# arkworks-rs/groth16

Measured on AMD Instinct MI355X. Metric: R1CS constraints/sec (create_proof, BLS12-381), higher is better.
Workload: dtype u32-limb Montgomery integers (Fr 255-bit, Fq 381-bit); 1 GPU; SYN(k=22) synthetic R1CS, 4194302 constraints, FFT domain 2^22, bls12_381, full create_proof (7 NTTs + 4 G1 MSMs + 1 G2 MSM), valid proving key generated on the GPU from seeded toxic waste; curve=bls12_381, log2_domain=22, constraints=4194302, key=valid, witness=resident in HBM at entry (--full: value_incl_h2d holds the PCIe-inclusive rates), parallelism=single-gpu

## Files before the change

### groth16_amd/csrc/api.hip

```cpp
#include "api_types.hpp"
#include "key_load.hpp"
#include "prover.hpp"
#include "proof_glue.hpp"
#include "unit_api.hpp"
#include "srs_setup.hpp"
#include "ceremony.hpp"

namespace {
template <class C>
struct Impl : KeyLoader<C>, Prover<C>, ProofGlue<C>, UnitApi<C> {
    typedef C Curve;
    typedef typename C::Fr Fr;
    typedef typename C::Fq Fq;
    typedef typename C::Fq2 Fq2;
};
}

#define G16_DISPATCH(curve, EXPR)                                             \
    do {                                                                      \
        try {                                                                 \
            if ((curve) == G16_BLS12_381) { typedef Impl<Bls12_381> I; return EXPR; } \
            if ((curve) == G16_BN254) { typedef Impl<Bn254> I; return EXPR; }  \
            return G16_ERR_BAD_ARG;                                           \
        } catch (const std::bad_alloc&) {                                     \
// ... 345 lines not shown
    }
    G16_HIP_TRY(hipSetDevice(ctx->device));
    G16_DISPATCH(ctx->curve, I::pk_load(ctx, view, out));
}

int g16_pk_load_bytes(g16_ctx* ctx, const uint8_t* bytes, uint64_t len, int compressed, int validate, g16_pk** out, void* info,
                      uint64_t info_size) {
    if (out) *out = nullptr;
    if (!ctx || !out || (!bytes && len) || (compressed != 0 && compressed != 1) || validate < 0 || validate > 2) return G16_ERR_BAD_ARG;
    if (!ctx->subs.empty()) {
        g_last_error = "g16_pk_load_bytes: the bytes of a key are loaded whole, on one GPU (a multi-device context takes g16_pk_load)";
        return G16_ERR_BAD_ARG;
    }
    return g16::pk_load_bytes(ctx, ctx->curve, ctx->device, ctx->stream, bytes, len, compressed, validate, out, info, info_size);
}

int g16_pk_load_bucket_shard(g16_ctx* ctx, const g16_pk_view* view, int rank, int world, g16_pk** out) {
    if (!ctx || !view || !out || world < 1 || world > 64 || rank < 0 || rank >= world) return G16_ERR_BAD_ARG;
    if (!ctx->subs.empty()) return G16_ERR_BAD_ARG;
    if (world == 1) return g16_pk_load(ctx, view, out);
    G16_HIP_TRY(hipSetDevice(ctx->device));
    G16_DISPATCH(ctx->curve, I::pk_load(ctx, view, out, world, rank));
}

int g16_pk_rebind_bucket_shard(g16_pk* pk, int rank, int world) {
    if (!pk || world < 1 || world > 64 || rank < 0 || rank >= world || !pk->subs.empty() || !pk->dp) return G16_ERR_BAD_ARG;
    auto rebind = [&](auto* dp) -> int {
        if (dp->c_z == 0 || dp->a_start || dp->b_g1_start || dp->b_g2_start || dp->h_start || dp->l_start) return G16_ERR_BAD_ARG;
        dp->shard_n = world;
        dp->shard_r = rank;
        return G16_OK;
    };
    if (pk->ctx->finprep.key_id == pk->id) pk->ctx->finprep.drop();
    pk->ctx->drop_prepared_sort(pk->id);
    if (pk->curve == G16_BLS12_381) return rebind(static_cast<DevicePk<Bls12_381>*>(pk->dp));
    return rebind(static_cast<DevicePk<Bn254>*>(pk->dp));
}

int g16_pk_get_info(const g16_pk* pk, g16_pk_info* out) {
    if (!pk || !out) return G16_ERR_BAD_ARG;
    memset(out, 0, sizeof(*out));
    const g16_pk* one = pk->subs.empty() ? pk : pk->subs[0];
    if (!one || !one->dp) return G16_ERR_BAD_ARG;
    auto fill = [&](const auto* dp) {
        out->window_bits_z = dp->c_z;
        out->window_bits_h = dp->c_h;
        out->table_fallback = dp->table_fallback;
        out->bucket_shard_rank = dp->shard_r;
        out->bucket_shard_world = dp->shard_n;
        out->device_bytes = dp->table_bytes;
    };
    if (one->curve == G16_BLS12_381) fill(static_cast<const DevicePk<Bls12_381>*>(one->dp));
    else fill(static_cast<const DevicePk<Bn254>*>(one->dp));
    out->n_devices = pk->subs.empty() ? 1 : (int)pk->subs.size();
    return G16_OK;
}

void g16_pk_free(g16_pk* pk) {
    if (!pk) return;
    if (!pk->ctx->subs.empty()) {
        for (g16_pk* sub : pk->subs) g16_pk_free(sub);
        delete pk;
        return;
    }
    if (pk->ctx->finprep.key_id == pk->id) pk->ctx->finprep.drop();
    (void)hipSetDevice(pk->ctx->device);
    pk->ctx->drop_prepared_sort(pk->id);
    if (pk->curve == G16_BLS12_381) Impl<Bls12_381>::pk_free(static_cast<DevicePk<Bls12_381>*>(pk->dp));
    else Impl<Bn254>::pk_free(static_cast<DevicePk<Bn254>*>(pk->dp));
    delete pk;
}

int g16_circuit_load(g16_ctx* ctx, const g16_csr_view abc[3], uint64_t num_inputs, uint64_t num_constraints, uint64_t num_variables,
                     g16_circuit** out) {
    return g16_circuit_load_qap(ctx, abc, num_inputs, num_constraints, num_variables, G16_QAP_LIBSNARK, out);
}

int g16_circuit_qap(const g16_circuit* c) { return c ? c->qap : -1; }

int g16_circuit_load_qap(g16_ctx* ctx, const g16_csr_view abc[3], uint64_t num_inputs, uint64_t num_constraints, uint64_t num_variables,
                         int qap, g16_circuit** out) {
    if (!ctx || !abc || !out) return G16_ERR_BAD_ARG;
    if (qap != G16_QAP_LIBSNARK && qap != G16_QAP_CIRCOM) return G16_ERR_BAD_ARG;
    if (!ctx->subs.empty()) {
        if (qap != G16_QAP_LIBSNARK) {
            g_last_error = "a Circom circuit cannot be loaded on a multi-device context (use one context per GPU and g16_prove_partial)";
            return G16_ERR_BAD_ARG;
        }
        const int n = (int)ctx->subs.size();
        g16_circuit* h = new (std::nothrow) g16_circuit{ctx->curve, ctx, nullptr, 0};
        if (!h) return G16_ERR_OOM;
        h->subs.assign((size_t)n, nullptr);
        const int rc = for_each_device(n, [&](int i) -> int {
            return g16_circuit_load(ctx->subs[(size_t)i], abc, num_inputs, num_constraints, num_variables, &h->subs[(size_t)i]);
        }, serial_loads(ctx));
        if (rc) { g16_circuit_free(h); return rc; }
        h->domain_size = h->subs[0]->domain_size;
        h->num_variables = num_variables;
// ... 727 lines not shown
```

### groth16_amd/csrc/api_types.hpp

```cpp
#pragma once
#include "internal.hpp"
#include "msm_common.hpp"
#include "fp30.hpp"
#include "fixed_base.hpp"
#include <atomic>
#include <chrono>
#include <condition_variable>
#include <future>
#include <mutex>
#include <thread>
#include <new>
#include <type_traits>
#include <dlfcn.h>

namespace g16 {

static thread_local std::string g_last_error;

void set_last_error(const char* what, hipError_t e, const char* file, int line) {
    char buf[512];
    snprintf(buf, sizeof(buf), "%s:%d: %s -> %s", file, line, what, hipGetErrorString(e));
    g_last_error = buf;
}

// ... 65 lines not shown
    hipEvent_t ev_up[8] = {};
    hipStream_t stream_wm = nullptr;
    hipEvent_t ev_dwm = nullptr;
    hipEvent_t ev_heavy[4] = {};
    hipEvent_t ev_edge[8] = {};
    struct Prepared {
        bool valid = false;
        const g16_pk* pk = nullptr;
        uint64_t key_id = 0;
        uint64_t a_start = 0, a_count = 0;
        int c_z = 0;
        const uint64_t* z = nullptr;
        uint64_t n_assign = 0;
        ScalarSort sort_z;
    } prep;
    void drop_prepared_sort(uint64_t id) {
        if (prep.valid && prep.key_id == id) { (void)hipStreamSynchronize(stream2); prep.valid = false; }
    }
    void reset_arena() {
        if (prep.valid) (void)hipStreamSynchronize(stream2);
        arena.reset();
        prep.valid = false;
    }
    hipStream_t red[5];
    Arena arena;
    g16_timings tm;
    g16_srs_timings srs_tm = {};
    double ceremony_ms[6] = {};
    double phase1_ms[5] = {};
    EventTimer t_wm, t_prep_h, t_prep_z, t_bucket[5], t_ntt[2];
    hipEvent_t ev_z = nullptr, ev_h = nullptr, ev_wm = nullptr, ev_done[5] = {};
    struct FinPrep {
        bool valid = false;
        std::future<void> fut;
        std::shared_ptr<void> data;
        uint64_t key_id = 0;
        uint64_t r[4] = {}, s[4] = {};
        bool matches(uint64_t id, const uint64_t* r_, const uint64_t* s_) const {
            return valid && key_id == id && memcmp(r, r_, 32) == 0 && memcmp(s, s_, 32) == 0;
        }
        void drop() {
            if (fut.valid()) fut.wait();
            valid = false;
            data.reset();
            key_id = 0;
        }
    } finprep;
    void* pinned = nullptr;
    size_t pinned_bytes = 0;
    uint64_t* check_z = nullptr;
    size_t check_z_bytes = 0;
    void* check_rec = nullptr;
    std::vector<g16_ctx*> subs;
    std::vector<char> peer;
};

struct DrainOnError {
    g16_ctx* ctx;
    bool armed = true;
    explicit DrainOnError(g16_ctx* c) : ctx(c) {}
    void dismiss() { armed = false; }
    ~DrainOnError() {
        if (!armed) return;
        (void)hipStreamSynchronize(ctx->stream);
        (void)hipStreamSynchronize(ctx->stream2);
        (void)hipStreamSynchronize(ctx->stream3);
        (void)hipStreamSynchronize(ctx->stream_wm);
        (void)hipStreamSynchronize(ctx->stream_h2d);
        for (int i = 0; i < 5; ++i) (void)hipStreamSynchronize(ctx->red[i]);
    }
};

struct g16_dwm;
struct DwmSlot {
    g16_dwm* dwm = nullptr;
    uint64_t *work[3] = {nullptr, nullptr, nullptr}, *recv[3] = {nullptr, nullptr, nullptr}, *h_local = nullptr;
    mutable uint64_t* h_full = nullptr;
    uint64_t* z_dev = nullptr;
};

// ... 76 lines not shown
```

### groth16_amd/csrc/internal.hpp

```cpp
#pragma once
#include <hip/hip_runtime.h>
#include <atomic>
#include <cstdint>
#include <cstdio>
#include <cstring>
#include <string>
#include <vector>
#include "../../include/g16_mi355x.h"
#include "curve.hpp"

namespace g16 {

void set_last_error(const char* what, hipError_t e, const char* file, int line);

#define G16_HIP_TRY(expr)                                                     \
    do {                                                                      \
        hipError_t e__ = (expr);                                              \
        if (e__ != hipSuccess) {                                              \
            ::g16::set_last_error(#expr, e__, __FILE__, __LINE__);            \
            return e__ == hipErrorOutOfMemory ? G16_ERR_OOM : G16_ERR_HIP;    \
        }                                                                     \
    } while (0)

#define G16_TRY(expr)                  \
// ... 168 lines not shown
    uint32_t max_segments = 0;
    uint64_t max_sorted = 0;
};
template <class C> int sort_scalars(const typename C::Fr* d_scalars, uint64_t n, int merged_c, Arena& arena, hipStream_t st, ScalarSort* out,
                                    int shard_n = 1, int shard_r = 0);
static constexpr int COEFF128_SWORDS = 7;
int coeffs128_plan(uint64_t n, MsmPlan* plan);
int sort_digit_planes(const MsmPlan& plan, const uint16_t* planes, uint64_t n, Arena& arena, hipStream_t st, ScalarSort* out);
int msm_slot_layout(const uint32_t* counts, uint32_t M, int R, uint32_t lseg, uint32_t* offsets, uint32_t* nparts, uint32_t* task_off,
                    uint32_t* heavy, uint32_t* block_sums, hipStream_t st);

template <class F>
struct MsmBuffers {
    void* partials = nullptr;
    void* chunk_out = nullptr;
    XYZZ<F>* window_sums = nullptr;
};
template <class F> int msm_bucket_pass(const Affine<F>* d_bases, int64_t shift, uint64_t base_count, const ScalarSort& ss, Arena& arena,
                                       hipStream_t st, MsmBuffers<F>* out, EventTimer* bucket_timer);
template <class F>
struct PassJob {
    const Affine<F>* bases;
    int64_t shift;
    uint64_t base_count;
    const ScalarSort* ss;
    MsmBuffers<F>* out;
};
template <class F> int msm_bucket_pass_batch(const PassJob<F>* jobs, int n, Arena& arena, hipStream_t st, EventTimer* bucket_timer);
template <class F> int msm_reduce(const MsmBuffers<F>& buf, const ScalarSort& ss, hipStream_t st);
template <class F> int msm_reduce_batch(const MsmBuffers<F>* const* bufs, const ScalarSort* const* sorts, int n, hipStream_t st, bool heavy_done);
template <class F> int msm_heavy_reduce(const MsmBuffers<F>& buf, const ScalarSort& ss, hipStream_t st);
template <class F> int msm_heavy_reduce_batch(const MsmBuffers<F>* const* bufs, const ScalarSort* const* sorts, int n, hipStream_t st);
template <class F> int convert_bases(Affine<F>* d_bases, uint64_t n, hipStream_t st);
template <class F> XYZZ<F> fold_windows(const XYZZ<F>* window_sums, const MsmPlan& plan);
template <class F> int build_window_tables(const Affine<F>* d_src, uint64_t n, int c, int W, Affine<F>* d_table, hipStream_t st, void* park = nullptr);
template <class F> size_t window_table_park_bytes(uint64_t n, int W);

template <class C>
int generate_parameters_device(hipStream_t st, Arena& arena, const g16_csr_view abc[3], uint64_t ni, uint64_t nc, uint64_t nv, int qap,
                               const g16_toxic_waste* tw, const uint64_t* g1_gen, const uint64_t* g2_gen, const g16_params_view* out);
template <class C>
int h_query_scalars_host(int qap, uint64_t domain_size, const uint64_t* t, const uint64_t* delta_inverse, uint64_t* out);
template <class C>
int qap_evaluations_host(const g16_csr_view abc[3], uint64_t ni, uint64_t nc, uint64_t nv, const uint64_t* t, uint64_t* a_out, uint64_t* b_out,
                         uint64_t* c_out, uint64_t* zt_out);

int serialize_points(int curve, int g2, int compressed, const uint64_t* points, uint64_t n, uint8_t* out);
int deserialize_points(int curve, int g2, int compressed, const uint8_t* in, uint64_t n, int validate, uint64_t* points_out);
uint64_t serialized_point_size(int curve, int g2, int compressed);

int pk_load_bytes(g16_ctx* ctx, int curve, int device, hipStream_t s, const uint8_t* bytes, uint64_t len, int compressed, int validate,
                  g16_pk** out, void* info_out, uint64_t info_size);

int mad_rate_device(hipStream_t st, double* mad_per_s);
template <class C> int synth_bases_device(int g2, uint64_t seed, uint64_t first, uint64_t n, void* out_dev, hipStream_t st);

}
```

### groth16_amd/csrc/msm.hip

```cpp
#include "internal.hpp"
#include "msm_common.hpp"
#include "fp30.hpp"
#include "acc_store.hpp"
#include "batch_affine.hpp"
#include "window_tables.hpp"
#include <algorithm>
#include <cstdlib>

namespace g16 {

static constexpr int SORT_THREADS = 1024;
static constexpr int RED_THREADS = 64;
static constexpr int WIN_THREADS = 256;
#ifndef G16_REDUCE_G
#define G16_REDUCE_G 8
#endif
static constexpr uint32_t REDUCE_G = G16_REDUCE_G;

struct PlanDev {
    int c, W;
    uint32_t B;
    uint32_t K[10];
    uint32_t shard_n, shard_r, shard_magic;
};

__device__ __forceinline__ bool shard_local_key(const PlanDev& plan, uint32_t* key) {
    if (plan.shard_n <= 1) return true;
    const uint32_t q = __umulhi(*key, plan.shard_magic);
    if (*key - q * plan.shard_n != plan.shard_r) return false;
    *key = q;
    return true;
}

template <class Fr>
__global__ __launch_bounds__(256) void digits_kernel(const Fr* __restrict__ scalars, uint64_t n, PlanDev plan,
                                                     uint16_t* __restrict__ planes) {
    __shared__ uint32_t sw[MSM_SWORDS][256];
    const uint64_t i = (uint64_t)blockIdx.x * 256 + threadIdx.x;
    if (i >= n) return;
    uint32_t s[Fr::N];
// ... 1251 lines not shown
    const MsmPlan& plan = sorts[0]->plan;
    for (int i = 1; i < n; ++i)
        if (sorts[i]->plan.B != plan.B || sorts[i]->plan.groups != plan.groups) return G16_ERR_INTERNAL;
    const uint32_t G = plan.chunk_buckets();
    const uint32_t cpw = plan.B / G;
    size_t lds_heavy, lds_win;
    G16_TRY(reduce_setup<F>(&lds_heavy, &lds_win));
    const auto batch = make_reduce_batch<F>(bufs, sorts, n);
    if (!heavy_done) G16_TRY((msm_heavy_reduce_batch<F>(bufs, sorts, n, st)));
    hipLaunchKernelGGL((bucket_reduce_kernel<F30>), dim3((cpw * plan.groups * F30::LANES_PER_TASK + RED_THREADS - 1) / RED_THREADS, n), dim3(RED_THREADS), 0,
                       st, batch, plan.B, plan.groups, G);
    G16_LAUNCH_CHECK();
    hipLaunchKernelGGL((window_reduce_kernel<F30>), dim3(plan.groups, plan.planes(), n), dim3(WIN_THREADS), lds_win, st, batch, cpw);
    G16_LAUNCH_CHECK();
    return G16_OK;
}

template <class F>
int msm_reduce(const MsmBuffers<F>& buf, const ScalarSort& ss, hipStream_t st) {
    const MsmBuffers<F>* b = &buf;
    const ScalarSort* s = &ss;
    return msm_reduce_batch<F>(&b, &s, 1, st, false);
}

template <class F>
int convert_bases(Affine<F>* d_bases, uint64_t n, hipStream_t st) {
    if (n == 0) return G16_OK;
    hipLaunchKernelGGL((convert_bases30_kernel<F>), dim3((unsigned)((n + 255) / 256)), dim3(256), 0, st, d_bases, n);
    G16_LAUNCH_CHECK();
    return G16_OK;
}

template <class F>
XYZZ<F> fold_windows(const XYZZ<F>* ws, const MsmPlan& plan) {
    const int NP = plan.planes(), bits = plan.chunk_bits();
    auto group_T = [&](int g) -> XYZZ<F> {
        const XYZZ<F>* P = ws + (size_t)g * NP;
        XYZZ<F> hi = XYZZ<F>::identity();
        for (int k = bits - 1; k >= 0; --k) { hi = hi.dbl(); hi.add(P[2 + k]); }
        for (uint32_t b = plan.chunk_buckets(); b > 1; b >>= 1) hi = hi.dbl();
        hi.add(P[0]);
        return hi;
    };
    XYZZ<F> total = XYZZ<F>::identity();
    if (plan.merged) {
        const int Q = plan.groups;
        if (Q > 1) {
            XYZZ<F> run = XYZZ<F>::identity();
            for (int q = Q - 1; q >= 1; --q) { run.add(ws[(size_t)q * NP + 1]); total.add(run); }
            for (uint32_t b = plan.B; b > 1; b >>= 1) total = total.dbl();
        }
        for (int q = 0; q < Q; ++q) total.add(group_T(q));
        if (plan.shard_n > 1) {
            XYZZ<F> plain = XYZZ<F>::identity();
            for (int q = 0; q < Q; ++q) plain.add(ws[(size_t)q * NP + 1]);
            const uint32_t kn = (uint32_t)plan.shard_n, km = (uint32_t)(plan.shard_n - 1 - plan.shard_r);
            total = total.mul_bits(&kn, 7);
            if (km) total.add(plain.mul_bits(&km, 7).neg());
        }
        return total;
    }
    for (int w = plan.W - 1; w >= 0; --w) {
        for (int k = 0; k < plan.c; ++k) total = total.dbl();
        total.add(group_T(w));
    }
    return total;
}

static constexpr int TABLE_MAX_W = 32;
static constexpr int TABLE_THREADS = 128;
static constexpr uint64_t TABLE_CHUNK = (uint64_t)1 << 18;
template <class F30>
__global__ __launch_bounds__(TABLE_THREADS, 2) void build_window_tables_kernel(const Affine<typename F30::Std>* __restrict__ src, uint64_t first,
                                                                              uint64_t count, uint64_t n, int c, int W,
                                                                              Affine<typename F30::Std>* __restrict__ table, uint32_t* __restrict__ park) {
    typedef TableDeviceIO<F30> IO;
    typedef typename IO::W32 W32;
    const uint64_t lane = (uint64_t)blockIdx.x * TABLE_THREADS + threadIdx.x;
    const uint64_t t = lane / F30::LANES_PER_TASK;
    if (t >= count) return;
    const uint64_t i = first + t;
    IO io{reinterpret_cast<const W32*>(src + i), reinterpret_cast<W32*>(table + i), n * 2 * IO::TL::PARTS, park + lane, count * F30::LANES_PER_TASK};
    window_table_task<F30>(io, c, W);
}

// ... 17 lines not shown
    for (uint64_t first = 0; first < n && rc == G16_OK; first += chunk) {
        const uint64_t count = std::min(chunk, n - first);
        const uint64_t lanes = count * F30::LANES_PER_TASK;
        hipLaunchKernelGGL((build_window_tables_kernel<F30>), dim3((unsigned)((lanes + TABLE_THREADS - 1) / TABLE_THREADS)), dim3(TABLE_THREADS), 0, st,
                           d_src, first, count, n, c, W, d_table, park);
        if (hipGetLastError() != hipSuccess) rc = G16_ERR_HIP;
    }
    if (!park_buf) {
        if (hipStreamSynchronize(st) != hipSuccess && rc == G16_OK) rc = G16_ERR_HIP;
        (void)hipFree(park);
    }
    return rc;
}

#define G16_INSTANTIATE_MSM(C)                                                                                               \
    template int convert_bases<typename C::Fq>(Affine<typename C::Fq>*, uint64_t, hipStream_t);                             \
    template int convert_bases<typename C::Fq2>(Affine<typename C::Fq2>*, uint64_t, hipStream_t);                           \
    template int sort_scalars<C>(const typename C::Fr*, uint64_t, int, Arena&, hipStream_t, ScalarSort*, int, int);                   \
    template int build_window_tables<typename C::Fq>(const Affine<typename C::Fq>*, uint64_t, int, int, Affine<typename C::Fq>*, hipStream_t, void*);    \
    template int build_window_tables<typename C::Fq2>(const Affine<typename C::Fq2>*, uint64_t, int, int, Affine<typename C::Fq2>*, hipStream_t, void*); \
    template size_t window_table_park_bytes<typename C::Fq>(uint64_t, int);                                                 \
    template size_t window_table_park_bytes<typename C::Fq2>(uint64_t, int);                                                \
    template int msm_bucket_pass<typename C::Fq>(const Affine<typename C::Fq>*, int64_t, uint64_t, const ScalarSort&, Arena&, \
                                                 hipStream_t, MsmBuffers<typename C::Fq>*, EventTimer*);                      \
    template int msm_bucket_pass<typename C::Fq2>(const Affine<typename C::Fq2>*, int64_t, uint64_t, const ScalarSort&,     \
                                                  Arena&, hipStream_t, MsmBuffers<typename C::Fq2>*, EventTimer*);            \
    template int msm_bucket_pass_batch<typename C::Fq>(const PassJob<typename C::Fq>*, int, Arena&, hipStream_t, EventTimer*);   \
    template int msm_bucket_pass_batch<typename C::Fq2>(const PassJob<typename C::Fq2>*, int, Arena&, hipStream_t, EventTimer*); \
    template int msm_reduce<typename C::Fq>(const MsmBuffers<typename C::Fq>&, const ScalarSort&, hipStream_t);             \
    template int msm_reduce_batch<typename C::Fq>(const MsmBuffers<typename C::Fq>* const*, const ScalarSort* const*, int, hipStream_t, bool); \
    template int msm_heavy_reduce<typename C::Fq>(const MsmBuffers<typename C::Fq>&, const ScalarSort&, hipStream_t);     \
    template int msm_heavy_reduce_batch<typename C::Fq>(const MsmBuffers<typename C::Fq>* const*, const ScalarSort* const*, int, hipStream_t); \
    template int msm_reduce<typename C::Fq2>(const MsmBuffers<typename C::Fq2>&, const ScalarSort&, hipStream_t);           \
    template XYZZ<typename C::Fq> fold_windows<typename C::Fq>(const XYZZ<typename C::Fq>*, const MsmPlan&);               \
    template XYZZ<typename C::Fq2> fold_windows<typename C::Fq2>(const XYZZ<typename C::Fq2>*, const MsmPlan&);

#if G16_MSM_PART == 0
G16_INSTANTIATE_MSM(Bls12_381)
#else
G16_INSTANTIATE_MSM(Bn254)
#endif

}
```

### groth16_amd/csrc/proof_glue.hpp

```cpp
#pragma once
#include "api_types.hpp"

namespace {

template <class C>
struct ProofGlue {
    typedef typename C::Fr Fr;
    typedef typename C::Fq Fq;
    typedef typename C::Fq2 Fq2;
    typedef typename C::G1A G1A;
    typedef typename C::G2A G2A;
    typedef typename C::G1X G1X;
    typedef typename C::G2X G2X;
    static constexpr int L = Fq::N / 2;
    struct FixedPoints {
        G1A alpha_g1, beta_g1, delta_g1, a_query0, b_g1_query0;
        G2A beta_g2, delta_g2, b_g2_query0;
    };
    struct FinalizePrep {
        G1X A0;
        G2X B2;
        G1X C0;
        uint32_t rk[Fr::N], sk[Fr::N];
        bool r_zero;
// ... 41 lines not shown
        G1X h_acc = G1X::identity(), l_acc = G1X::identity(), a_msm = G1X::identity(), b1_msm = G1X::identity();
        G2X b2_msm = G2X::identity();
        for (int i = 0; i < n_parts; ++i) {
            h_acc.add(load_xyzz<G1X>(parts[i].h));
            l_acc.add(load_xyzz<G1X>(parts[i].l));
            a_msm.add(load_xyzz<G1X>(parts[i].a));
            b1_msm.add(load_xyzz<G1X>(parts[i].b_g1));
            b2_msm.add(load_xyzz<G2X>(parts[i].b_g2));
        }
        auto fut_b2 = std::async(std::launch::async, [&]() {
            G2X g2_b = fp.B2;
            g2_b.add(b2_msm);
            return g2_b.to_affine();
        });
        const bool need_rb1 = !fp.r_zero && !b1_msm.is_identity();
        std::future<G1X> fut_rb1;
        if (need_rb1) fut_rb1 = std::async(std::launch::async, [&]() { return mul_window4(b1_msm, fp.rk); });
        G1X g_a = fp.A0;
        g_a.add(a_msm);
        G1X g_c = fp.C0;
        g_c.add(mul_window4(a_msm, fp.sk));
        g_c.add(l_acc);
        g_c.add(h_acc);
        if (need_rb1) g_c.add(fut_rb1.get());
        G1A pa, pc;
        two_to_affine(g_a, g_c, &pa, &pc);
        const G2A pb = fut_b2.get();
        memset(out, 0, sizeof(*out));
        memcpy(out->a, &pa, sizeof(pa));
        memcpy(out->b, &pb, sizeof(pb));
        memcpy(out->c, &pc, sizeof(pc));
        return G16_OK;
    }
    static int finalize_core(const FixedPoints& pk, const g16_partial* parts, int n_parts, const uint64_t* r_, const uint64_t* s_,
                             g16_proof* out, const FixedBaseTable<G1X>* d1 = nullptr, const FixedBaseTable<G2X>* d2 = nullptr) {
        if (n_parts < 1) return G16_ERR_BAD_ARG;
        return finalize_finish(finalize_prepare_core(pk, r_, s_, d1, d2), parts, n_parts, out);
    }
    static FixedPoints fixed_points(const KeyGlue<C>* pk) {
        return {pk->alpha_g1, pk->beta_g1, pk->delta_g1, pk->a_query0, pk->b_g1_query0, pk->beta_g2, pk->delta_g2, pk->b_g2_query0};
    }
    static void ensure_delta_tables(KeyGlue<C>* pk) {
        std::lock_guard<std::mutex> lk(pk->tab_mu);
        if (!pk->tabs_ready.load(std::memory_order_relaxed) && ++pk->finalize_calls >= 2) {
            auto f1 = std::async(std::launch::async, [&]() { pk->delta1_tab.build(G1X::from_affine(pk->delta_g1)); });
            pk->delta2_tab.build(G2X::from_affine(pk->delta_g2));
            f1.get();
            pk->tabs_ready.store(true, std::memory_order_release);
        }
    }
    static const FixedBaseTable<G1X>* table1(const KeyGlue<C>* pk) { return pk->tabs_ready.load(std::memory_order_acquire) ? &pk->delta1_tab : nullptr; }
    static const FixedBaseTable<G2X>* table2(const KeyGlue<C>* pk) { return pk->tabs_ready.load(std::memory_order_acquire) ? &pk->delta2_tab : nullptr; }
    static int prove_finalize_prepare(g16_ctx* ctx, const g16_pk* pkh, const uint64_t* r_, const uint64_t* s_) {
        const std::shared_ptr<KeyGlue<C>> glue = static_cast<const DevicePk<C>*>(pkh->dp)->glue;
        ctx->finprep.drop();
        auto data = std::make_shared<FinalizePrep>();
        ctx->finprep.data = data;
        ctx->finprep.key_id = pkh->id;
        memcpy(ctx->finprep.r, r_, 32);
        memcpy(ctx->finprep.s, s_, 32);
        struct RS { uint64_t r[4], s[4]; } rs;
        memcpy(rs.r, r_, 32);
        memcpy(rs.s, s_, 32);
        ctx->finprep.fut = std::async(std::launch::async, [glue, data, rs]() {
            ensure_delta_tables(glue.get());
            *data = finalize_prepare_core(fixed_points(glue.get()), rs.r, rs.s, table1(glue.get()), table2(glue.get()));
        });
        ctx->finprep.valid = true;
        return G16_OK;
    }
    static int prove_finalize(g16_ctx* ctx, const g16_pk* pkh, const g16_partial* parts, int n_parts, const uint64_t* r_, const uint64_t* s_,
                              g16_proof* out) {
        KeyGlue<C>* pk = static_cast<const DevicePk<C>*>(pkh->dp)->glue.get();
        const double t0 = now_ms();
        if (n_parts < 1) return G16_ERR_BAD_ARG;
        if (ctx->finprep.matches(pkh->id, r_, s_)) {
            ctx->finprep.fut.get();
            const std::shared_ptr<void> keep = ctx->finprep.data;
            ctx->finprep.valid = false;
            G16_TRY(finalize_finish(*static_cast<const FinalizePrep*>(keep.get()), parts, n_parts, out));
        } else {
            ensure_delta_tables(pk);
            G16_TRY(finalize_core(fixed_points(pk), parts, n_parts, r_, s_, out, table1(pk), table2(pk)));
        }
        const double dt = now_ms() - t0;
        ctx->tm.finish_ms += dt;
        ctx->tm.total_ms += dt;
        return G16_OK;
    }
    static int finalize_host(const g16_pk_view* v, const g16_partial* parts, int n_parts, const uint64_t* r_, const uint64_t* s_,
                             g16_proof* out) {
        if (!v->alpha_g1 || !v->beta_g1 || !v->delta_g1 || !v->beta_g2 || !v->delta_g2 || !v->a_query0 || !v->b_g1_query0 ||
            !v->b_g2_query0)
            return G16_ERR_BAD_ARG;
        const FixedPoints fp = {load_pod<G1A>(v->alpha_g1), load_pod<G1A>(v->beta_g1), load_pod<G1A>(v->delta_g1), load_pod<G1A>(v->a_query0),
                                load_pod<G1A>(v->b_g1_query0), load_pod<G2A>(v->beta_g2), load_pod<G2A>(v->delta_g2),
                                load_pod<G2A>(v->b_g2_query0)};
        return finalize_core(fp, parts, n_parts, r_, s_, out);
    }

};

}
```

### groth16_amd/csrc/prover.hpp

```cpp
#pragma once
#include "api_types.hpp"

namespace {

template <class C>
struct Prover {
    typedef typename C::Fr Fr;
    typedef typename C::Fq Fq;
    typedef typename C::Fq2 Fq2;
    typedef typename C::G1A G1A;
    typedef typename C::G2A G2A;
    typedef typename C::G1X G1X;
    typedef typename C::G2X G2X;
    static constexpr int L = Fq::N / 2;
    static int stage_assignment(g16_ctx* ctx, const uint64_t* z, uint64_t n_assign, int on_device, const Fr** d_z) {
        if (on_device) { *d_z = reinterpret_cast<const Fr*>(z); return G16_OK; }
        Fr* buf = nullptr;
        G16_TRY(ctx->arena.alloc_n(n_assign, &buf));
        G16_HIP_TRY(hipMemcpyAsync(buf, z, n_assign * sizeof(Fr), hipMemcpyHostToDevice, ctx->stream));
        *d_z = buf;
        return G16_OK;
    }


    static int prove_partial_prepare(g16_ctx* ctx, const g16_pk* pkh, const g16_circuit* ckh, const uint64_t* z_dev, uint64_t n_assign) {
        const DevicePk<C>* pk = static_cast<const DevicePk<C>*>(pkh->dp);
        const DeviceCircuit<C>* ck = static_cast<const DeviceCircuit<C>*>(ckh->dc);
        if (n_assign != ck->num_variables) return G16_ERR_BAD_LENGTH;
        if (pk->a_start + pk->a_count > n_assign - 1) return G16_ERR_BAD_LENGTH;
        DrainOnError drain(ctx);
        ctx->reset_arena();
        const Fr* d_z = reinterpret_cast<const Fr*>(z_dev);
        ScalarSort ss;
        G16_TRY((sort_scalars<C>(d_z + 1 + pk->a_start, pk->a_count, pk->c_z, ctx->arena, ctx->stream2, &ss, pk->shard_n, pk->shard_r)));
        G16_HIP_TRY(hipEventRecord(ctx->ev_z, ctx->stream2));
        ctx->prep.valid = true;
        ctx->prep.pk = pkh;
        ctx->prep.key_id = pkh->id;
        ctx->prep.a_start = pk->a_start;
        ctx->prep.a_count = pk->a_count;
        ctx->prep.c_z = pk->c_z;
        ctx->prep.z = z_dev;
        ctx->prep.n_assign = n_assign;
        ctx->prep.sort_z = ss;
        drain.dismiss();
        return G16_OK;
    }

    static int prove_partial(g16_ctx* ctx, const g16_pk* pkh, const g16_circuit* ckh, const uint64_t* z, uint64_t n_assign, int on_device,
                             int skip_b_g1, g16_partial* out, const Fr* h_ext = nullptr, uint64_t h_ext_len = 0) {
        const DevicePk<C>* pk = static_cast<const DevicePk<C>*>(pkh->dp);
        const DeviceCircuit<C>* ck = static_cast<const DeviceCircuit<C>*>(ckh->dc);
        hipStream_t s1 = ctx->stream, s2 = ctx->stream2, s3 = ctx->stream3;
        if (n_assign != ck->num_variables) return G16_ERR_BAD_LENGTH;
        const uint64_t n = ck->dom->n, nin = ck->num_inputs;
        const uint64_t m = n_assign - 1, w = n_assign - nin;
        if (pk->a_start + pk->a_count > m || pk->l_start + pk->l_count > w || pk->h_start + pk->h_count > (h_ext ? h_ext_len : n))
            return G16_ERR_BAD_LENGTH;
        if (pk->b_g1_start != pk->a_start || pk->b_g1_count != pk->a_count || pk->b_g2_start != pk->a_start ||
            pk->b_g2_count != pk->a_count)
            return G16_ERR_BAD_ARG;
        memset(out, 0, sizeof(*out));
        const double t_begin = now_ms();
        DrainOnError drain(ctx);
        const bool prepared = ctx->prep.valid && on_device && ctx->prep.pk == pkh && ctx->prep.key_id == pkh->id && ctx->prep.z == z &&
                              ctx->prep.n_assign == n_assign && ctx->prep.a_start == pk->a_start && ctx->prep.a_count == pk->a_count &&
                              ctx->prep.c_z == pk->c_z && ctx->prep.sort_z.plan.shard_n == pk->shard_n &&
                              ctx->prep.sort_z.plan.shard_r == pk->shard_r;
        const ScalarSort prepared_sort = ctx->prep.sort_z;
        if (prepared) ctx->prep.valid = false;
        else ctx->reset_arena();
        const Fr* d_z = nullptr;
        ZUpload up;
        const bool chunked = !on_device && !h_ext && !prepared && !(getenv("G16_UPLOAD_CHUNKED") && atoi(getenv("G16_UPLOAD_CHUNKED")) == 0);
        if (chunked) {
            Fr* buf = nullptr;
            G16_TRY(ctx->arena.alloc_n(n_assign, &buf));
            d_z = buf;
            up.host = z;
            up.copy_stream = ctx->stream_h2d;
            for (int i = 0; i < 8; ++i) up.landed[i] = ctx->ev_up[i];
        } else {
            G16_TRY(stage_assignment(ctx, z, n_assign, on_device, &d_z));
            if (!prepared) G16_HIP_TRY(hipEventRecord(ctx->ev_z, s1));
        }

        const bool overlap_map = !h_ext && getenv("G16_MAP_UNDER_PASSES") != nullptr && atoi(getenv("G16_MAP_UNDER_PASSES")) != 0;
        hipStream_t sm = overlap_map ? ctx->stream_wm : s1;
        Fr* d_h = nullptr;
        ScalarSort sort_h, sort_z, sort_l;
        if (overlap_map && !chunked) G16_HIP_TRY(hipStreamWaitEvent(sm, ctx->ev_z, 0));
        G16_TRY(ctx->t_wm.start(sm));
        if (h_ext) {
            d_h = const_cast<Fr*>(h_ext);
            ctx->t_ntt[0].used = ctx->t_ntt[1].used = false;
// ... 62 lines not shown
        };

        const bool l_covered = pk->l_count == 0 || (pk->l_start + nin - 1 >= pk->a_start &&
                                                    pk->l_start + pk->l_count + nin - 1 <= pk->a_start + pk->a_count);
        {
            hipStream_t sr = short_passes ? ctx->red[4] : s2;
            RoctxRange rr("Compute B in G2");
            if (concurrent) {
                G16_HIP_TRY(hipStreamWaitEvent(sr, ctx->ev_z, 0));
                G16_HIP_TRY(hipStreamWaitEvent(sr, ctx->ev_wm, 0));
                G16_TRY(run_pass(4, pk->b_g2, 0, pk->b_g2_count, sort_z, &buf_b2, sr));
            } else {
                G16_TRY(run_pass(4, pk->b_g2, 0, pk->b_g2_count, sort_z, &buf_b2));
                G16_HIP_TRY(hipStreamWaitEvent(sr, pass_end[4], 0));
            }
            G16_TRY((msm_reduce(buf_b2, sort_z, sr)));
            G16_TRY(copy_out(4, buf_b2, sort_z, sr));
        }
        struct G1Job { int k; MsmBuffers<Fq>* buf; const ScalarSort* ss; };
        G1Job jobs[4];
        int njobs = 0;
        PassJob<Fq> pj[4];
        int pk_of[4], npj = 0;
        double weight[5] = {0, 0, 0, 0, 0};
        auto plans_match = [](const MsmPlan& x, const MsmPlan& y) {
            return x.B == y.B && x.groups == y.groups && x.Lmax == y.Lmax && x.merged == y.merged && x.affine_levels == 0 && y.affine_levels == 0;
        };
        const bool batch_ok = sort_z.plan.affine_levels == 0 || sort_z.max_sorted == 0;
        bool h_in_batch = h_ext != nullptr && batch_ok && plans_match(sort_z.plan, sort_h.plan) && !getenv("G16_PASS_NO_BATCH");
        if (const char* e = getenv("G16_PASS_H_IN_BATCH")) h_in_batch = h_in_batch && atoi(e) != 0;
        int g1_launches = 0;
        bool last_batch = false, early[4] = {false, false, false, false};
        int early_ev[4] = {0, 1, 2, 3};
        auto run_batch = [&]() -> int {
            if (!npj) return G16_OK;
            hipEvent_t b0, b1;
            if (last_end) b0 = last_end;
            else G16_TRY(mark(&b0));
            if (batch_ok && !getenv("G16_PASS_NO_BATCH")) {
                G16_TRY((msm_bucket_pass_batch<Fq>(pj, npj, ctx->arena, s1, nullptr)));
                ++g1_launches;
            } else {
                for (int i = 0; i < npj; ++i) {
                    G16_TRY((msm_bucket_pass<Fq>(pj[i].bases, pj[i].shift, pj[i].base_count, *pj[i].ss, ctx->arena, s1, pj[i].out, nullptr)));
                    ++g1_launches;
                }
            }
            G16_TRY(mark(&b1));
            last_end = b1;
            for (int i = 0; i < npj; ++i) { pass_begin[pk_of[i]] = b0; pass_end[pk_of[i]] = b1; }
            if (!last_batch) {
                const MsmBuffers<Fq>* eb[4];
                const ScalarSort* es[4];
                for (int i = 0; i < npj; ++i) { eb[i] = pj[i].out; es[i] = pj[i].ss; }
                const int k0 = pk_of[0];
                G16_HIP_TRY(hipStreamWaitEvent(ctx->red[k0], b1, 0));
                if (batch_ok) {
                    G16_TRY((msm_heavy_reduce_batch<Fq>(eb, es, npj, ctx->red[k0])));
                } else {
                    for (int i = 0; i < npj; ++i) G16_TRY((msm_heavy_reduce<Fq>(*eb[i], *es[i], ctx->red[k0])));
                }
                G16_HIP_TRY(hipEventRecord(ctx->ev_heavy[k0], ctx->red[k0]));
                for (int i = 0; i < npj; ++i) { early[pk_of[i]] = true; early_ev[pk_of[i]] = k0; }
            }
            npj = 0;
            return G16_OK;
        };
        auto queue_pass = [&](int k, const G1A* bases, int64_t shift, uint64_t count, const ScalarSort& ss, MsmBuffers<Fq>* buf) {
            pj[npj] = PassJob<Fq>{bases, shift, count, &ss, buf};
            pk_of[npj++] = k;
            weight[k] = (double)count;
            jobs[njobs++] = {k, buf, &ss};
        };
        if (l_covered) {
            const int64_t shift = (int64_t)pk->a_start - (int64_t)(nin - 1) - (int64_t)pk->l_start;
            queue_pass(1, pk->l, shift, pk->l_count, sort_z, &buf_l);
        } else {
            G16_TRY((sort_scalars<C>(d_z + nin + pk->l_start, pk->l_count, pk->c_z, ctx->arena, s1, &sort_l, pk->shard_n, pk->shard_r)));
            last_end = nullptr;
            queue_pass(1, pk->l, 0, pk->l_count, sort_l, &buf_l);
            G16_TRY(run_batch());
        }
        { RoctxRange rr("Compute A");
        queue_pass(2, pk->a, 0, pk->a_count, sort_z, &buf_a); }
        if (!skip_b_g1) {
            RoctxRange rr("Compute B in G1");
            queue_pass(3, pk->b_g1, 0, pk->b_g1_count, sort_z, &buf_b1);
        }
        if (!h_in_batch) G16_TRY(run_batch());
        G16_HIP_TRY(hipStreamWaitEvent(s1, ctx->ev_h, 0));
        if (!h_in_batch) last_end = nullptr;
        { RoctxRange rr("Compute C");
        queue_pass(0, pk->h, 0, pk->h_count, sort_h, &buf_h);
        last_batch = true;
        G16_TRY(run_batch()); }
        bool done[4] = {false, false, false, false};
        for (int i = 0; i < njobs; ++i) {
            if (done[i]) continue;
            const MsmBuffers<Fq>* bb[4];
            const ScalarSort* sp[4];
            int idx[4], nb = 0;
            for (int q = i; q < njobs; ++q)
                if (!done[q] && jobs[q].ss->plan.B == jobs[i].ss->plan.B && jobs[q].ss->plan.groups == jobs[i].ss->plan.groups) {
                    bb[nb] = jobs[q].buf; sp[nb] = jobs[q].ss; idx[nb] = q; ++nb;
                    done[q] = true;
                }
            bool any_early = false;
            for (int q = 0; q < nb; ++q) any_early = any_early || early[jobs[idx[q]].k];
            for (int q = 0; q < nb; ++q) {
                if (early[jobs[idx[q]].k]) G16_HIP_TRY(hipStreamWaitEvent(s1, ctx->ev_heavy[early_ev[jobs[idx[q]].k]], 0));
                else if (any_early) G16_TRY((msm_heavy_reduce<Fq>(*bb[q], *sp[q], s1)));
            }
            G16_TRY((msm_reduce_batch<Fq>(bb, sp, nb, s1, any_early)));
            for (int q = 0; q < nb; ++q) G16_TRY(copy_out(jobs[idx[q]].k, *jobs[idx[q]].buf, *jobs[idx[q]].ss, s1));
        }

        double fold_ms = 0.0;
        {
            G16_HIP_TRY(hipEventSynchronize(ctx->ev_done[4]));
            const double t0 = now_ms();
            store_xyzz(out->b_g2, fold_windows<Fq2>(reinterpret_cast<const G2X*>(pin + 4 * SLOT), sort_z.plan));
            fold_ms += now_ms() - t0;
        }
        if (skip_b_g1) store_xyzz(out->b_g1, G1X::identity());
        {
            for (int q = 0; q < njobs; ++q) G16_HIP_TRY(hipEventSynchronize(ctx->ev_done[jobs[q].k]));
            const double t0 = now_ms();
            struct FoldJob { int k; const MsmPlan* plan; uint64_t* dst; };
            const FoldJob fj[4] = {{1, l_covered ? &sort_z.plan : &sort_l.plan, out->l}, {2, &sort_z.plan, out->a}, {3, &sort_z.plan, out->b_g1},
                                   {0, &sort_h.plan, out->h}};
            auto fold_one = [&](const FoldJob& f) { store_xyzz(f.dst, fold_windows<Fq>(reinterpret_cast<const G1X*>(pin + f.k * SLOT), *f.plan)); };
            std::future<void> fut[3];
            int nf = 0;
            for (int q = 0; q < 3; ++q) {
                if (fj[q].k == 3 && skip_b_g1) continue;
                const FoldJob f = fj[q];
                fut[nf++] = std::async(std::launch::async, [&fold_one, f]() { fold_one(f); });
            }
            fold_one(fj[3]);
            for (int q = 0; q < nf; ++q) fut[q].get();
            fold_ms += now_ms() - t0;
        }
        G16_HIP_TRY(hipStreamSynchronize(s1));
        G16_HIP_TRY(hipStreamSynchronize(s2));
        G16_HIP_TRY(hipStreamSynchronize(s3));
        if (overlap_map) G16_HIP_TRY(hipStreamSynchronize(ctx->stream_wm));
        for (int k = 0; k < 5; ++k) G16_HIP_TRY(hipStreamSynchronize(ctx->red[k]));
        drain.dismiss();
        const double t_end = now_ms();

        g16_timings& tm = ctx->tm;
        memset(&tm, 0, sizeof(tm));
        auto span = [&](int k) -> double {
            float t = 0.f;
            return (pass_begin[k] && hipEventElapsedTime(&t, pass_begin[k], ctx->ev_done[k]) == hipSuccess) ? (double)t : 0.0;
        };
        tm.witness_map_ms = ctx->t_wm.ms();
        tm.ntt_ms = ctx->t_ntt[0].ms() + ctx->t_ntt[1].ms();
        tm.scalar_prep_ms = ctx->t_prep_h.ms() + ctx->t_prep_z.ms();
        tm.msm_h_ms = span(0);
        tm.msm_l_ms = span(1);
        tm.msm_a_ms = span(2);
        tm.msm_b_g1_ms = skip_b_g1 ? 0.0 : span(3);
        tm.msm_b_g2_ms = span(4);
        for (int i = 0; i < 5; ++i) {
            float t = 0.f;
            tm.bucket_ms[i] = (pass_begin[i] && pass_end[i] && hipEventElapsedTime(&t, pass_begin[i], pass_end[i]) == hipSuccess) ? (double)t : 0.0;
            double wsum = 0.0;
            for (int q = 0; q < 4; ++q) if (pass_begin[q] == pass_begin[i] && pass_end[q] == pass_end[i]) wsum += weight[q];
            if (i < 4 && wsum > 0.0) tm.bucket_ms[i] *= weight[i] / wsum;
            tm.bucket_pass_ms += tm.bucket_ms[i];
        }
        tm.g1_pass_launches = (double)g1_launches;
        tm.finish_ms = fold_ms;
        tm.total_ms = t_end - t_begin;
        tm.window_bits = sort_z.plan.c;
        tm.windows = sort_z.plan.W;
        return G16_OK;
    }

};
// ... 3 lines not shown
```

Baseline: 66.69 million constraints/s.

## Overlap host window folds and proof glue with remaining GPU MSM work

When the whole key is on one device, the light G1 MSM reductions are now finished and copied out early on the reduce streams. Two worker threads fold the G2 and G1 window sums, with multithreaded fold_windows, and compute the A, B and partial C glue while the H MSM is still running on the GPU. The glue result is cached in a FinCache keyed by key id, r, s and the partial sums, so finalize only adds H and converts C to affine. This adds host threads, more synchronisation complexity and cache-invalidation paths.

```diff
diff --git a/groth16_amd/csrc/api.hip b/groth16_amd/csrc/api.hip
--- a/groth16_amd/csrc/api.hip
+++ b/groth16_amd/csrc/api.hip
@@ -401,6 +401,7 @@
         return G16_OK;
     };
     if (pk->ctx->finprep.key_id == pk->id) pk->ctx->finprep.drop();
+    if (pk->ctx->fincache.key_id == pk->id) pk->ctx->fincache.drop();
     pk->ctx->drop_prepared_sort(pk->id);
     if (pk->curve == G16_BLS12_381) return rebind(static_cast<DevicePk<Bls12_381>*>(pk->dp));
     return rebind(static_cast<DevicePk<Bn254>*>(pk->dp));
@@ -433,6 +434,7 @@
         return;
     }
     if (pk->ctx->finprep.key_id == pk->id) pk->ctx->finprep.drop();
+    if (pk->ctx->fincache.key_id == pk->id) pk->ctx->fincache.drop();
     (void)hipSetDevice(pk->ctx->device);
     pk->ctx->drop_prepared_sort(pk->id);
     if (pk->curve == G16_BLS12_381) Impl<Bls12_381>::pk_free(static_cast<DevicePk<Bls12_381>*>(pk->dp));
diff --git a/groth16_amd/csrc/api_types.hpp b/groth16_amd/csrc/api_types.hpp
--- a/groth16_amd/csrc/api_types.hpp
+++ b/groth16_amd/csrc/api_types.hpp
@@ -121,7 +121,7 @@
     hipEvent_t ev_z = nullptr, ev_h = nullptr, ev_wm = nullptr, ev_done[5] = {};
     struct FinPrep {
         bool valid = false;
-        std::future<void> fut;
+        std::shared_future<void> fut;
         std::shared_ptr<void> data;
         uint64_t key_id = 0;
         uint64_t r[4] = {}, s[4] = {};
@@ -135,6 +135,19 @@
             key_id = 0;
         }
     } finprep;
+    struct FinCache {
+        std::atomic<bool> ready{false};
+        uint64_t key_id = 0;
+        uint64_t r[4] = {}, s[4] = {};
+        g16_partial part = {};
+        uint64_t a[12] = {}, b[24] = {};
+        uint64_t c_part[24] = {};
+        void drop() { ready.store(false, std::memory_order_release); key_id = 0; }
+        bool matches(uint64_t id, const uint64_t* r_, const uint64_t* s_, const g16_partial* p, int n_parts) const {
+            return n_parts == 1 && ready.load(std::memory_order_acquire) && key_id == id && memcmp(r, r_, 32) == 0 && memcmp(s, s_, 32) == 0 &&
+                   memcmp(&part, p, sizeof(g16_partial)) == 0;
+        }
+    } fincache;
     void* pinned = nullptr;
     size_t pinned_bytes = 0;
     uint64_t* check_z = nullptr;
diff --git a/groth16_amd/csrc/internal.hpp b/groth16_amd/csrc/internal.hpp
--- a/groth16_amd/csrc/internal.hpp
+++ b/groth16_amd/csrc/internal.hpp
@@ -224,7 +224,7 @@
 template <class F> int msm_heavy_reduce(const MsmBuffers<F>& buf, const ScalarSort& ss, hipStream_t st);
 template <class F> int msm_heavy_reduce_batch(const MsmBuffers<F>* const* bufs, const ScalarSort* const* sorts, int n, hipStream_t st);
 template <class F> int convert_bases(Affine<F>* d_bases, uint64_t n, hipStream_t st);
-template <class F> XYZZ<F> fold_windows(const XYZZ<F>* window_sums, const MsmPlan& plan);
+template <class F> XYZZ<F> fold_windows(const XYZZ<F>* window_sums, const MsmPlan& plan, int threads = 1);
 template <class F> int build_window_tables(const Affine<F>* d_src, uint64_t n, int c, int W, Affine<F>* d_table, hipStream_t st, void* park = nullptr);
 template <class F> size_t window_table_park_bytes(uint64_t n, int W);
 
diff --git a/groth16_amd/csrc/msm.hip b/groth16_amd/csrc/msm.hip
--- a/groth16_amd/csrc/msm.hip
+++ b/groth16_amd/csrc/msm.hip
@@ -6,6 +6,7 @@
 #include "window_tables.hpp"
 #include <algorithm>
 #include <cstdlib>
+#include <future>
 
 namespace g16 {
 
@@ -1323,7 +1324,7 @@
 }
 
 template <class F>
-XYZZ<F> fold_windows(const XYZZ<F>* ws, const MsmPlan& plan) {
+XYZZ<F> fold_windows(const XYZZ<F>* ws, const MsmPlan& plan, int threads) {
     const int NP = plan.planes(), bits = plan.chunk_bits();
     auto group_T = [&](int g) -> XYZZ<F> {
         const XYZZ<F>* P = ws + (size_t)g * NP;
@@ -1341,7 +1342,20 @@
             for (int q = Q - 1; q >= 1; --q) { run.add(ws[(size_t)q * NP + 1]); total.add(run); }
             for (uint32_t b = plan.B; b > 1; b >>= 1) total = total.dbl();
         }
-        for (int q = 0; q < Q; ++q) total.add(group_T(q));
+        const int nt = threads < 1 ? 1 : (threads > Q ? Q : threads);
+        if (nt > 1) {
+            auto range_T = [&](int t) {
+                XYZZ<F> acc = XYZZ<F>::identity();
+                for (int q = (int)((int64_t)Q * t / nt); q < (int)((int64_t)Q * (t + 1) / nt); ++q) acc.add(group_T(q));
+                return acc;
+            };
+            std::vector<std::future<XYZZ<F>>> fut;
+            for (int t = 1; t < nt; ++t) fut.push_back(std::async(std::launch::async, range_T, t));
+            total.add(range_T(0));
+            for (auto& f : fut) total.add(f.get());
+        } else {
+            for (int q = 0; q < Q; ++q) total.add(group_T(q));
+        }
         if (plan.shard_n > 1) {
             XYZZ<F> plain = XYZZ<F>::identity();
             for (int q = 0; q < Q; ++q) plain.add(ws[(size_t)q * NP + 1]);
@@ -1425,8 +1439,8 @@
     template int msm_heavy_reduce<typename C::Fq>(const MsmBuffers<typename C::Fq>&, const ScalarSort&, hipStream_t);     \
     template int msm_heavy_reduce_batch<typename C::Fq>(const MsmBuffers<typename C::Fq>* const*, const ScalarSort* const*, int, hipStream_t); \
     template int msm_reduce<typename C::Fq2>(const MsmBuffers<typename C::Fq2>&, const ScalarSort&, hipStream_t);           \
-    template XYZZ<typename C::Fq> fold_windows<typename C::Fq>(const XYZZ<typename C::Fq>*, const MsmPlan&);               \
-    template XYZZ<typename C::Fq2> fold_windows<typename C::Fq2>(const XYZZ<typename C::Fq2>*, const MsmPlan&);
+    template XYZZ<typename C::Fq> fold_windows<typename C::Fq>(const XYZZ<typename C::Fq>*, const MsmPlan&, int);              \
+    template XYZZ<typename C::Fq2> fold_windows<typename C::Fq2>(const XYZZ<typename C::Fq2>*, const MsmPlan&, int);
 
 #if G16_MSM_PART == 0
 G16_INSTANTIATE_MSM(Bls12_381)
diff --git a/groth16_amd/csrc/proof_glue.hpp b/groth16_amd/csrc/proof_glue.hpp
--- a/groth16_amd/csrc/proof_glue.hpp
+++ b/groth16_amd/csrc/proof_glue.hpp
@@ -97,6 +97,44 @@
         memcpy(out->c, &pc, sizeof(pc));
         return G16_OK;
     }
+    struct EarlyGlue {
+        G1A a;
+        G2A b;
+        G1X c_part;
+    };
+    static G2A early_b(const FinalizePrep& fp, const G2X& b2_msm) {
+        G2X g2_b = fp.B2;
+        g2_b.add(b2_msm);
+        return g2_b.to_affine();
+    }
+    static void early_ac(const FinalizePrep& fp, const G1X& l_acc, const G1X& a_msm, const G1X& b1_msm, G1A* pa, G1X* c_part) {
+        const bool need_rb1 = !fp.r_zero && !b1_msm.is_identity();
+        std::future<G1X> fut_rb1;
+        if (need_rb1) fut_rb1 = std::async(std::launch::async, [&]() { return mul_window4(b1_msm, fp.rk); });
+        *c_part = fp.C0;
+        c_part->add(mul_window4(a_msm, fp.sk));
+        c_part->add(l_acc);
+        if (need_rb1) c_part->add(fut_rb1.get());
+        G1X g_a = fp.A0;
+        g_a.add(a_msm);
+        *pa = g_a.to_affine();
+    }
+    static EarlyGlue finalize_early(const FinalizePrep& fp, const G1X& l_acc, const G1X& a_msm, const G1X& b1_msm, const G2X& b2_msm) {
+        EarlyGlue eg;
+        auto fut_b2 = std::async(std::launch::async, [&]() { return early_b(fp, b2_msm); });
+        early_ac(fp, l_acc, a_msm, b1_msm, &eg.a, &eg.c_part);
+        eg.b = fut_b2.get();
+        return eg;
+    }
+    static void finalize_late(const G1A& pa, const G2A& pb, const G1X& c_part, const G1X& h_acc, g16_proof* out) {
+        G1X g_c = c_part;
+        g_c.add(h_acc);
+        const G1A pc = g_c.to_affine();
+        memset(out, 0, sizeof(*out));
+        memcpy(out->a, &pa, sizeof(pa));
+        memcpy(out->b, &pb, sizeof(pb));
+        memcpy(out->c, &pc, sizeof(pc));
+    }
     static int finalize_core(const FixedPoints& pk, const g16_partial* parts, int n_parts, const uint64_t* r_, const uint64_t* s_,
                              g16_proof* out, const FixedBaseTable<G1X>* d1 = nullptr, const FixedBaseTable<G2X>* d2 = nullptr) {
         if (n_parts < 1) return G16_ERR_BAD_ARG;
@@ -139,7 +177,14 @@
         KeyGlue<C>* pk = static_cast<const DevicePk<C>*>(pkh->dp)->glue.get();
         const double t0 = now_ms();
         if (n_parts < 1) return G16_ERR_BAD_ARG;
-        if (ctx->finprep.matches(pkh->id, r_, s_)) {
+        if (ctx->fincache.matches(pkh->id, r_, s_, parts, n_parts)) {
+            if (ctx->finprep.matches(pkh->id, r_, s_)) {
+                ctx->finprep.fut.get();
+                ctx->finprep.valid = false;
+            }
+            const g16_ctx::FinCache& fc = ctx->fincache;
+            finalize_late(load_pod<G1A>(fc.a), load_pod<G2A>(fc.b), load_xyzz<G1X>(fc.c_part), load_xyzz<G1X>(parts[0].h), out);
+        } else if (ctx->finprep.matches(pkh->id, r_, s_)) {
             ctx->finprep.fut.get();
             const std::shared_ptr<void> keep = ctx->finprep.data;
             ctx->finprep.valid = false;
@@ -161,6 +206,12 @@
         const FixedPoints fp = {load_pod<G1A>(v->alpha_g1), load_pod<G1A>(v->beta_g1), load_pod<G1A>(v->delta_g1), load_pod<G1A>(v->a_query0),
                                 load_pod<G1A>(v->b_g1_query0), load_pod<G2A>(v->beta_g2), load_pod<G2A>(v->delta_g2),
                                 load_pod<G2A>(v->b_g2_query0)};
+        if (n_parts == 1) {
+            const EarlyGlue eg = finalize_early(finalize_prepare_core(fp, r_, s_), load_xyzz<G1X>(parts[0].l), load_xyzz<G1X>(parts[0].a),
+                                                load_xyzz<G1X>(parts[0].b_g1), load_xyzz<G2X>(parts[0].b_g2));
+            finalize_late(eg.a, eg.b, eg.c_part, load_xyzz<G1X>(parts[0].h), out);
+            return G16_OK;
+        }
         return finalize_core(fp, parts, n_parts, r_, s_, out);
     }
 
diff --git a/groth16_amd/csrc/prover.hpp b/groth16_amd/csrc/prover.hpp
--- a/groth16_amd/csrc/prover.hpp
+++ b/groth16_amd/csrc/prover.hpp
@@ -1,5 +1,6 @@
 #pragma once
 #include "api_types.hpp"
+#include "proof_glue.hpp"
 
 namespace {
 
@@ -61,6 +62,7 @@
             pk->b_g2_count != pk->a_count)
             return G16_ERR_BAD_ARG;
         memset(out, 0, sizeof(*out));
+        ctx->fincache.drop();
         const double t_begin = now_ms();
         DrainOnError drain(ctx);
         const bool prepared = ctx->prep.valid && on_device && ctx->prep.pk == pkh && ctx->prep.key_id == pkh->id && ctx->prep.z == z &&
@@ -189,6 +191,9 @@
         int g1_launches = 0;
         bool last_batch = false, early[4] = {false, false, false, false};
         int early_ev[4] = {0, 1, 2, 3};
+        const bool whole_key = pk->shard_n == 1 && pk->a_start == 0 && pk->a_count == m && pk->l_start == 0 && pk->l_count == w && pk->h_start == 0;
+        const bool early_sums = whole_key && !h_ext && !h_in_batch && batch_ok && !getenv("G16_PASS_NO_BATCH");
+        bool reduced[4] = {false, false, false, false};
         auto run_batch = [&]() -> int {
             if (!npj) return G16_OK;
             hipEvent_t b0, b1;
@@ -217,8 +222,16 @@
                 } else {
                     for (int i = 0; i < npj; ++i) G16_TRY((msm_heavy_reduce<Fq>(*eb[i], *es[i], ctx->red[k0])));
                 }
-                G16_HIP_TRY(hipEventRecord(ctx->ev_heavy[k0], ctx->red[k0]));
-                for (int i = 0; i < npj; ++i) { early[pk_of[i]] = true; early_ev[pk_of[i]] = k0; }
+                if (early_sums) {
+                    G16_TRY((msm_reduce_batch<Fq>(eb, es, npj, ctx->red[k0], true)));
+                    for (int i = 0; i < npj; ++i) {
+                        G16_TRY(copy_out(pk_of[i], *pj[i].out, *pj[i].ss, ctx->red[k0]));
+                        reduced[pk_of[i]] = true;
+                    }
+                } else {
+                    G16_HIP_TRY(hipEventRecord(ctx->ev_heavy[k0], ctx->red[k0]));
+                    for (int i = 0; i < npj; ++i) { early[pk_of[i]] = true; early_ev[pk_of[i]] = k0; }
+                }
             }
             npj = 0;
             return G16_OK;
@@ -245,6 +258,64 @@
             queue_pass(3, pk->b_g1, 0, pk->b_g1_count, sort_z, &buf_b1);
         }
         if (!h_in_batch) G16_TRY(run_batch());
+        struct Workers {
+            std::thread th[2];
+            int rc[2] = {G16_OK, G16_OK};
+            std::string err[2];
+            bool glued = false;
+            typename ProofGlue<C>::EarlyGlue eg;
+            void join() { for (auto& t : th) if (t.joinable()) t.join(); }
+            ~Workers() { join(); }
+        } workers;
+        if (skip_b_g1) store_xyzz(out->b_g1, G1X::identity());
+        if (early_sums) {
+            typedef ProofGlue<C> Glue;
+            const bool with_glue = ctx->finprep.valid && ctx->finprep.key_id == pkh->id && ctx->finprep.data && ctx->finprep.fut.valid();
+            const typename Glue::FinalizePrep* fp = with_glue ? static_cast<const typename Glue::FinalizePrep*>(ctx->finprep.data.get()) : nullptr;
+            const std::shared_future<void> prep_done = ctx->finprep.fut;
+            workers.glued = with_glue;
+            auto run = [&workers](int i, auto body) {
+                workers.th[i] = std::thread([&workers, i, body]() {
+                    workers.rc[i] = body();
+                    if (workers.rc[i] != G16_OK) workers.err[i] = g_last_error;
+                });
+            };
+            run(0, [&, fp, prep_done]() -> int {
+                G16_HIP_TRY(hipSetDevice(ctx->device));
+                G16_HIP_TRY(hipEventSynchronize(ctx->ev_done[4]));
+                const G2X b2 = fold_windows<Fq2>(reinterpret_cast<const G2X*>(pin + 4 * SLOT), sort_z.plan, 6);
+                store_xyzz(out->b_g2, b2);
+                if (fp) {
+                    prep_done.wait();
+                    workers.eg.b = Glue::early_b(*fp, b2);
+                }
+                return G16_OK;
+            });
+            run(1, [&, fp, prep_done]() -> int {
+                G16_HIP_TRY(hipSetDevice(ctx->device));
+                auto fold_g1 = [&](int k) {
+                    const MsmPlan& plan = (k == 1 && !l_covered) ? sort_l.plan : sort_z.plan;
+                    uint64_t* dst = k == 1 ? out->l : k == 2 ? out->a : out->b_g1;
+                    store_xyzz(dst, fold_windows<Fq>(reinterpret_cast<const G1X*>(pin + k * SLOT), plan, 2));
+                };
+                if (!l_covered) {
+                    G16_HIP_TRY(hipEventSynchronize(ctx->ev_done[1]));
+                    fold_g1(1);
+                }
+                G16_HIP_TRY(hipEventSynchronize(ctx->ev_done[skip_b_g1 ? 2 : 3]));
+                std::future<void> fut[2];
+                int nf = 0;
+                if (l_covered) fut[nf++] = std::async(std::launch::async, fold_g1, 1);
+                if (!skip_b_g1) fut[nf++] = std::async(std::launch::async, fold_g1, 3);
+                fold_g1(2);
+                for (int q = 0; q < nf; ++q) fut[q].get();
+                if (fp) {
+                    prep_done.wait();
+                    Glue::early_ac(*fp, load_xyzz<G1X>(out->l), load_xyzz<G1X>(out->a), load_xyzz<G1X>(out->b_g1), &workers.eg.a, &workers.eg.c_part);
+                }
+                return G16_OK;
+            });
+        }
         G16_HIP_TRY(hipStreamWaitEvent(s1, ctx->ev_h, 0));
         if (!h_in_batch) last_end = nullptr;
         { RoctxRange rr("Compute C");
@@ -252,6 +323,7 @@
         last_batch = true;
         G16_TRY(run_batch()); }
         bool done[4] = {false, false, false, false};
+        for (int i = 0; i < njobs; ++i) done[i] = reduced[jobs[i].k];
         for (int i = 0; i < njobs; ++i) {
             if (done[i]) continue;
             const MsmBuffers<Fq>* bb[4];
@@ -273,14 +345,24 @@
         }
 
         double fold_ms = 0.0;
-        {
-            G16_HIP_TRY(hipEventSynchronize(ctx->ev_done[4]));
+        if (early_sums) {
+            G16_HIP_TRY(hipEventSynchronize(ctx->ev_done[0]));
             const double t0 = now_ms();
-            store_xyzz(out->b_g2, fold_windows<Fq2>(reinterpret_cast<const G2X*>(pin + 4 * SLOT), sort_z.plan));
-            fold_ms += now_ms() - t0;
-        }
-        if (skip_b_g1) store_xyzz(out->b_g1, G1X::identity());
-        {
+            store_xyzz(out->h, fold_windows<Fq>(reinterpret_cast<const G1X*>(pin), sort_h.plan, 4));
+            workers.join();
+            for (int i = 0; i < 2; ++i)
+                if (workers.rc[i] != G16_OK) {
+                    g_last_error = workers.err[i];
+                    return workers.rc[i];
+                }
+            fold_ms = now_ms() - t0;
+        } else {
+            {
+                G16_HIP_TRY(hipEventSynchronize(ctx->ev_done[4]));
+                const double t0 = now_ms();
+                store_xyzz(out->b_g2, fold_windows<Fq2>(reinterpret_cast<const G2X*>(pin + 4 * SLOT), sort_z.plan));
+                fold_ms += now_ms() - t0;
+            }
             for (int q = 0; q < njobs; ++q) G16_HIP_TRY(hipEventSynchronize(ctx->ev_done[jobs[q].k]));
             const double t0 = now_ms();
             struct FoldJob { int k; const MsmPlan* plan; uint64_t* dst; };
@@ -304,6 +386,19 @@
         if (overlap_map) G16_HIP_TRY(hipStreamSynchronize(ctx->stream_wm));
         for (int k = 0; k < 5; ++k) G16_HIP_TRY(hipStreamSynchronize(ctx->red[k]));
         drain.dismiss();
+        if (workers.glued) {
+            g16_ctx::FinCache& fc = ctx->fincache;
+            fc.key_id = pkh->id;
+            memcpy(fc.r, ctx->finprep.r, 32);
+            memcpy(fc.s, ctx->finprep.s, 32);
+            memcpy(&fc.part, out, sizeof(*out));
+            memset(fc.a, 0, sizeof(fc.a));
+            memset(fc.b, 0, sizeof(fc.b));
+            memcpy(fc.a, &workers.eg.a, sizeof(workers.eg.a));
+            memcpy(fc.b, &workers.eg.b, sizeof(workers.eg.b));
+            store_xyzz(fc.c_part, workers.eg.c_part);
+            fc.ready.store(true, std::memory_order_release);
+        }
         const double t_end = now_ms();
 
         g16_timings& tm = ctx->tm;
```

After: 66.99 million constraints/s (median of 6 runs). About the same (+0.5%).
